# TencentYoutuResearch/ImageMatching-OETR

Hardware: AMD Instinct MI355X
Metric: image-pairs/sec @640x640 (OETR hot path: feature correlation + overlap regression, features resident in HBM) (higher is better)
Workload: dtype f32 (3xf16-split operands, fp32 accumulate); 1 GPU; BASELINE configs[1]: batch=8 pairs/GPU, 640x640 -> 20x20 tokens/image, C=256, 8 enc + 2 dec layers, f32_split_f16; pairs_per_gpu=8, global_pairs=8, streams=3, world_size=1, gpu_max_hw_queues=4, encoder_tile_rows=64, tail_mode=direct form (throughput setting for overlapped streams), parallelism=pairs sharded over 1 rank(s); all-gather of boxes only

## Files before the change

imagematching_oetr_amd/csrc/api.hip:

```cpp
#include <math.h>
#include <stdlib.h>
#include <string.h>

#include <atomic>
#include <string>
#include <vector>

#include "../../include/oetr_hip.h"
#include "../../include/oetr_tail_share.h"
#include "common.h"

using namespace oetr;

constexpr int OETR_PREREDUCE_MIN_TOKENS = 768;
constexpr int OETR_DIRECT_TAIL_MIN_ROWS = 16000;

namespace {

thread_local std::string g_err;

oetr_status fail(oetr_status st, const std::string& msg) {
  g_err = msg;
  return st;
}
// ... 103 lines not shown
  std::vector<hipEvent_t> ev;
  std::vector<int> kid;
  int used = 0;
  int dropped = 0;
};

struct oetr_ctx {
  oetr_trace* trace = nullptr;
  int device = 0;
  int mode = GM_SPLIT;
  int kv_prereduce = -1;
  int tail_share = -1;
  mutable std::atomic<int> enc_grid{0};
  mutable int dec_fault = 0;
  int dec_split = 0;
  int tail_mode = 0;
  int policy = 0;
  int enc_tile = 0;
  int attn_full = 0;
  int num_cus = 256;
  float* dev = nullptr;
  size_t dev_floats = 0;
  EncLayerDev enc[OETR_N_ENC];
  DecKVDev dkv;
  DecLayerDev dec[OETR_N_DEC];
  const float* qe[2];
  const float *dec_tgt1, *dec_q0, *dec_qkv1;
  HeadsDev heads;
};

struct oetr_neck_ctx {
  oetr_trace* trace = nullptr;
  int device = 0;
  int num_cus = 256;
  int conv_rows = 0;
  float* dev = nullptr;
  const f32x4 *proj_wh[2], *proj_wl[2];
  const float *proj_b, *ln_w, *ln_b;
  const f32x4 *conv_wh[3], *conv_wl[3];
  const f32x4 *conv_wh_rw[3], *conv_wl_rw[3];
  int conv_kernel = 0;
  const float* conv_b[3];
  const f32x4 *out_wh, *out_wl;
  const float* out_b;
};

namespace {

#ifdef OETR_PHASE_TIMING
long long* g_tbuf = nullptr;
#endif

struct Workspace {
  float *x, *qp, *pos, *kvp[2], *ksp[2], *att0, *z0, *dkv1, *dks1, *conv_out, *gn_part, *sm_part, *hs,
      *logits, *cxy, *tlbr, *convp, *kbuf[2], *vt[2], *kvr, *ksr;
  uint32_t* flags;
  size_t bytes;
};

bool make_geom(int n, int hf1, int wf1, int hf2, int wf2, Geom* g) {
  if (n <= 0 || hf1 <= 0 || wf1 <= 0 || hf2 <= 0 || wf2 <= 0) return false;
  const long L1 = (long)hf1 * wf1, L2 = (long)hf2 * wf2;
  if (L1 > OETR_MAX_TOKENS || L2 > OETR_MAX_TOKENS) return false;
  if ((long)n * (L1 + L2) > (1L << 30) / C) return false;
  g->N = n;
  g->L[0] = (int)L1; g->L[1] = (int)L2;
  g->hf[0] = hf1; g->wf[0] = wf1; g->hf[1] = hf2; g->wf[1] = wf2;
  g->nt[0] = (g->L[0] + TM - 1) / TM; g->nt[1] = (g->L[1] + TM - 1) / TM;
  g->row0[0] = 0; g->row0[1] = n * g->L[0];
  g->prow0[0] = 0; g->prow0[1] = g->L[0];
  g->tile0[0] = 0; g->tile0[1] = n * g->nt[0];
  g->ntiles = n * (g->nt[0] + g->nt[1]);
  g->rows = n * (g->L[0] + g->L[1]);
  return true;
}

int encoder_tile_rows(const oetr_ctx* h, const Geom& g) {
  if (!gm_half(h->mode) || h->attn_full) return TM;
  const int want = h->enc_tile;
  if (want == TM || want == 64) return want;
  return g.ntiles > h->num_cus ? 64 : TM;
}
Geom encoder_geom(const Geom& g, int rows) {
  Geom e = g;
  for (int i = 0; i < 2; ++i) e.nt[i] = (g.L[i] + rows - 1) / rows;
  e.tile0[0] = 0; e.tile0[1] = g.N * e.nt[0];
  e.ntiles = g.N * (e.nt[0] + e.nt[1]);
  return e;
}

Workspace carve(const Geom& g, void* base, bool attn_full = false) {
  Workspace w;
  size_t off = 0;
  auto take = [&](size_t floats) {
    float* p = base ? reinterpret_cast<float*>(static_cast<char*>(base) + off) : nullptr;
    off += (floats * sizeof(float) + 255) & ~size_t(255);
    return p;
  };
  const size_t rows = g.rows, nt = g.ntiles;
  w.flags = reinterpret_cast<uint32_t*>(take(OETR_WORKSPACE_STATUS_BYTES / sizeof(float)));
  w.x = take(rows * C);
  w.qp = take((rows + (size_t)2 * g.N * 64) * C);
  w.pos = take((size_t)(g.L[0] + g.L[1]) * C);
  for (int i = 0; i < 2; ++i) { w.kvp[i] = take(nt * KV_FLOATS); w.ksp[i] = take(nt * C); }
  w.att0 = take(nt * C); w.z0 = take(nt * NH);
  w.dkv1 = take(nt * KV_FLOATS); w.dks1 = take(nt * C);
  w.conv_out = take(rows * C);
  w.gn_part = take(nt * 32 * 2);
  w.sm_part = take(nt * 4);
  w.hs = take((size_t)2 * g.N * C);
  w.logits = take(rows);
  w.cxy = take((size_t)2 * g.N * 2);
  w.tlbr = take((size_t)2 * g.N * 4);
  w.convp = take((size_t)9 * rows * C);
  w.kvr = take((size_t)2 * g.N * KV_FLOATS);
  w.ksr = take((size_t)2 * g.N * C);
  for (int i = 0; i < 2; ++i) {
    w.kbuf[i] = attn_full ? take(rows * C) : nullptr;
    w.vt[i] = attn_full ? take((size_t)g.N * C * TM * (g.nt[0] + g.nt[1])) : nullptr;
  }
  w.bytes = off;
  return w;
}

oetr_status check_ws(const Geom& g, void* ws, size_t ws_bytes, Workspace* out, bool attn_full = false) {
  if (!ws) return fail(OETR_ERR_WORKSPACE, "workspace is NULL");
  if (reinterpret_cast<uintptr_t>(ws) & 255)
    return fail(OETR_ERR_WORKSPACE, "workspace must be 256-byte aligned");
  *out = carve(g, ws, attn_full);
  if (out->bytes > ws_bytes)
    return fail(OETR_ERR_WORKSPACE, "workspace too small: need " + std::to_string(out->bytes) +
                                        " bytes, got " + std::to_string(ws_bytes));
  return OETR_OK;
}

HeatLaunch heat_launch(const oetr_ctx* h, const Geom& g, const Workspace& w, const float* mem1,
                       const float* mem2, const float* hs1, const float* hs2, float* cxy1,
                       float* cxy2, int img_h1, int img_h2) {
  HeatLaunch p;
  p.g = g;
  p.w = h->heads;
  p.mem[0] = mem1; p.mem[1] = mem2;
  p.hs[0] = hs1; p.hs[1] = hs2;
  p.conv_out = w.conv_out;
  p.gn_part = w.gn_part;
  p.sm_part = w.sm_part;
  p.logits = w.logits;
  p.cxy[0] = cxy1; p.cxy[1] = cxy2;
  p.img_h[0] = img_h1; p.img_h[1] = img_h2;
  p.tlbr[0] = p.tlbr[1] = nullptr;
  p.box[0] = p.box[1] = nullptr;
  p.img_w[0] = p.img_w[1] = 0;
  p.flags = w.flags;
  p.publish = nullptr;
  p.force_staged_conv = h->tail_mode == 3;
  p.convp_units = 9;
  p.mask[0] = p.mask[1] = nullptr;
  return p;
}

oetr_status check_masks(const oetr_ctx* h, const float* mask1, const float* mask2, bool encoder) {
  if (!mask1 && !mask2) return OETR_OK;
  if (!mask1 || !mask2) return fail(OETR_ERR_BAD_ARG, "masks: pass both mask1 and mask2, or neither");
  if (encoder && ((h->mode != GM_SPLIT && h->mode != GM_F32) || h->attn_full))
    return fail(OETR_ERR_UNSUPPORTED, "masks: built for OETR_DTYPE_F32_SPLIT_F16, OETR_DTYPE_F32_SPLIT_QK16 and OETR_DTYPE_F32 with linear attention "
                                      "(the reference's FullAttention turns a masked query row into NaN, "
                                      "linear_attention.py:74-81)");
  return OETR_OK;
}

struct Scoped {
  oetr_trace* t; hipStream_t s; int slot;
  Scoped(oetr_trace* tr, hipStream_t s_, int kid) : t(tr), s(s_), slot(-1) {
// ... 26 lines not shown
      const int units = 9 * g.N * ((g.L[0] + RT - 1) / RT + (g.L[1] + RT - 1) / RT);
      const int avail = h->num_cus - images * DEC_SPLIT_K;
      const int upi = std::max(3, (units + avail - 1) / avail);
      fits = upi <= 9;
      if (fits) d.convp_units = upi;
    } else {
      fits = images * DEC_SPLIT_K + g.ntiles <= h->num_cus;
    }
  }
  if (h->dec_split == DEC_SPLIT_K && d.convp_units == 9 && beside_convp && gm_half(h->mode)) d.convp_units = 3;
  d.ksplit = (h->dec_split == DEC_SPLIT_K || (h->dec_split == 0 && fits)) && images <= DEC_SPLIT_MAX_IMAGES
                 ? DEC_SPLIT_K : 1;
  d.flags = w.flags;
  d.xch_epoch = w.flags + STATUS_EPOCH_WORD;
  d.xch = reinterpret_cast<unsigned long long*>(reinterpret_cast<char*>(w.flags) + STATUS_XCH_OFFSET);
  d.tbuf = nullptr;
  d.dbg = 0;
  if (d.ksplit == DEC_SPLIT_K && h->dec_fault) { d.dbg = DEC_DBG_FAULT; h->dec_fault = 0; }
#ifdef OETR_PHASE_TIMING
  d.tbuf = g_tbuf ? g_tbuf + 16 * 4096 : nullptr;
#endif
  return d;
}

oetr_status run_correlation(oetr_ctx* h, const Geom& g, const Workspace& w, const float* feat1,
                            const float* feat2, const float* pos1, const float* pos2,
                            int enc_layers, hipStream_t s, bool with_decoder = true,
                            bool resident = false, const float* mask1 = nullptr,
                            const float* mask2 = nullptr) {
  EncLaunch p;
  memset(&p, 0, sizeof(p));
  if (!resident) {
    p.feat_nchw[0] = feat1; p.feat_nchw[1] = feat2;
    p.pos_nchw[0] = pos1; p.pos_nchw[1] = pos2;
    p.pos_out = w.pos;
  }
  p.tile_rows = encoder_tile_rows(h, g);
  p.g = encoder_geom(g, p.tile_rows);
  p.tail_share = h->tail_share != 0;
  p.attn_full = h->attn_full;
  h->enc_grid.store(encoder_workgroups(p, h->mode), std::memory_order_relaxed);
#ifdef OETR_ABLATE
  { const char* e = getenv("OETR_ABLATE"); p.dbg = e ? atoi(e) : 0; }
#endif
#ifdef OETR_PHASE_TIMING
  {
    static long long* tb = nullptr;
    if (!tb) (void)hipMalloc(&tb, sizeof(long long) * 16 * 65536);
    p.tbuf = tb;
    g_tbuf = tb;
  }
#endif
  p.x = w.x; p.qp = w.qp; p.pos = w.pos;
  p.mask[0] = mask1; p.mask[1] = mask2;
  p.flags = w.flags;
  p.policy = h->policy;
  for (int i = 0; i < 2; ++i) p.lpad[i] = g.nt[i] * TM;
  p.vt_off[0] = 0; p.vt_off[1] = (size_t)g.N * C * p.lpad[0];
  p.kbuf_out = w.kbuf[0]; p.vt_out = w.vt[0];
  p.a = h->enc[0];
  p.kv_out = w.kvp[0]; p.ks_out = w.ksp[0];
  int prereduce = h->attn_full ? 0 : h->kv_prereduce;
  if (prereduce < 0) prereduce = (g.L[0] >= OETR_PREREDUCE_MIN_TOKENS || g.L[1] >= OETR_PREREDUCE_MIN_TOKENS) ? 1 : 0;
  TRACED(h, s, K_ENC_A, launch_encoder(p, false, 0, h->mode, s));
  p.feat_nchw[0] = p.feat_nchw[1] = p.pos_nchw[0] = p.pos_nchw[1] = nullptr;
  for (int l = 0; l < enc_layers; ++l) {
    p.b = h->enc[l];
    p.b_cross = l & 1;
    p.kv_in = w.kvp[l & 1]; p.ks_in = w.ksp[l & 1];
    p.kv_reduced = 0;
    if (prereduce == 1) {
      TRACED(h, s, K_KV_REDUCE, launch_kv_reduce(p.g, w.kvp[l & 1], w.ksp[l & 1], w.kvr, w.ksr, s));
      p.kv_in = w.kvr; p.ks_in = w.ksr;
      p.kv_reduced = 1;
    }
    p.kbuf_in = w.kbuf[l & 1]; p.vt_in = w.vt[l & 1];
    int tail;
    if (l + 1 == OETR_N_ENC) {
      tail = 1;
      p.d = h->dkv;
      p.att0_out = w.att0; p.z0_out = w.z0; p.dkv1_out = w.dkv1; p.dks1_out = w.dks1;
      p.dec_q0 = h->dec_q0;
    } else if (l + 1 < enc_layers) {
      tail = 0;
      p.a = h->enc[l + 1];
      p.kv_out = w.kvp[(l + 1) & 1]; p.ks_out = w.ksp[(l + 1) & 1];
      p.kbuf_out = w.kbuf[(l + 1) & 1]; p.vt_out = w.vt[(l + 1) & 1];
    } else {
      tail = 2;
    }
    TRACED(h, s, tail == 0 ? K_ENC_BA : tail == 1 ? K_ENC_BDEC : K_ENC_B,
           launch_encoder(p, true, tail, h->mode, s));
  }
  if (enc_layers == OETR_N_ENC && with_decoder) {
    DecLaunch d = dec_launch(h, g, w);
    TRACED(h, s, K_DECODER, launch_decoder(d, s));
  }
  return OETR_OK;
}

oetr_status check_weight(const char* name, const float* w, size_t n, bool f16_range) {
  for (size_t i = 0; i < n; ++i) {
    const float a = fabsf(w[i]);
    if (!(a <= 3.4028234e38f))
      return fail(OETR_ERR_UNSUPPORTED, std::string(name) + ": non-finite weight at index " + std::to_string(i));
    if (f16_range && a >= 65504.0f)
// ... 1034 lines not shown
```

imagematching_oetr_amd/csrc/common.h:

```cpp
#pragma once
#include <hip/hip_runtime.h>
#include <stdint.h>

#include <string>
#include <type_traits>

#include "../../include/oetr_hip.h"

namespace oetr {

constexpr int C = 256;
constexpr int NH = 8;
constexpr int HD = 32;
constexpr int FF = 512;
constexpr int TM = 32;
constexpr int LDA = C + 4;
constexpr int LDH = FF + 4;
constexpr int NTHREADS = 256;
constexpr int KV_FLOATS = NH * HD * HD;
constexpr float LN_EPS = 1e-5f;
constexpr float ATTN_EPS = 1e-6f;
constexpr int MAX_TOKENS = 10000;


// ... 759 lines not shown
    NoEpi none;
    gemm_epi<KTOT, P, HAS_NEXT, NKTOT, SITE, NSITE, TR>(A, W, Wl, nt0, ks0, lane, acc, nW, nWl, nnt0,
                                                        nks0, none);
  }
  template <int KTOT, int P, bool HAS_NEXT, int NKTOT, int SITE = SITE_FULL, int NSITE = SITE_FULL,
            bool TR = false, class EPI, int RP>
  __device__ __forceinline__ void gemm_epi(const PlanesT<M, RP>& A, const f32x4* W, const f32x4* Wl, int nt0,
                                           int ks0, int lane, f32x16 (&acc)[NMT], const f32x4* nW,
                                           const f32x4* nWl, int nnt0, int nks0, EPI& epi) {
    const size_t off = ((size_t)nt0 * (KTOT / 16) + ks0) * 64;
    const size_t noff = ((size_t)nnt0 * (NKTOT / 16) + nks0) * 64;
    const int a_off = (lane & 31) * LDAH + 8 * (lane >> 5);
    const _Float16* ah_ptr = A.h + a_off;
    const _Float16* al_ptr = A.l + a_off;
    AStep a[2];
    load_a<SITE>(a[0], ah_ptr, al_ptr, 0);
    f32x16 cross[NMT];
#pragma unroll
    for (int mt = 0; mt < NMT; ++mt) cross[mt] = f32x16{0};
    step<P, HAS_NEXT, 0, EPI, TR, SITE, NSITE>(ah_ptr, al_ptr, W + off, Wl + off,
                                               HAS_NEXT ? nW + noff : nullptr,
                                               HAS_NEXT ? nWl + noff : nullptr, a, acc, cross, epi);
    if constexpr (TWO && SITE != SITE_HI) {
#pragma unroll
      for (int mt = 0; mt < NMT; ++mt)
#pragma unroll
        for (int r = 0; r < 16; ++r) acc[mt][r] = fmaf(cross[mt][r], SPLIT_INV, acc[mt][r]);
    }
  }
};
typedef WStream2T<GM_SPLIT> WStream2;

#endif

int set_last_error(int status, const char* msg);
oetr_status entry_fail(const char* entry, oetr_status status, const std::string& msg);
oetr_status entry_hip(const char* entry, hipError_t e, const char* what);
hipError_t clear_i32(int32_t* p, int64_t n, hipStream_t s);
struct EncLayerDev {
  const f32x4 *wq, *wk, *wv, *wmerge, *w1, *w2;
  const f32x4 *wq_l, *wk_l, *wv_l, *wmerge_l, *w1_l, *w2_l;
  const float *lnq_w, *lnq_b, *lnkv_w, *lnkv_b, *ln2_w, *ln2_b;
};
struct DecKVDev {
  const f32x4 *wk[2], *wv[2];
  const f32x4 *wk_l[2], *wv_l[2];
  const float *bk[2], *bv[2];
};

struct EncLaunch {
  Geom g;
  float* x;
  float* qp;
  const float* pos;
  const float* kv_in;
  const float* ks_in;
  float* kv_out;
  float* ks_out;
  float* att0_out;
  float* z0_out;
  float* dkv1_out;
  float* dks1_out;
  const float* dec_q0;
  EncLayerDev b;
  EncLayerDev a;
  DecKVDev d;
  int attn_full;
  const float* kbuf_in;
  const float* vt_in;
  float* kbuf_out;
  float* vt_out;
  int lpad[2];
  size_t vt_off[2];
  int tile_rows;
  int nwg;
  int tail_share;
  int b_cross;
  int kv_reduced;
  int policy;
  int dbg;
  long long* tbuf;
  uint32_t* flags;
  const float* feat_nchw[2];
  const float* pos_nchw[2];
  float* pos_out;
  const float* mask[2];
};

hipError_t launch_encoder(const EncLaunch& p, bool has_b, int tail, int mode, hipStream_t s);
int encoder_workgroups(const EncLaunch& p, int mode);
hipError_t launch_kv_reduce(const Geom& g, const float* kvp, const float* ksp, float* kvr, float* ksr,
                            hipStream_t s);

struct MhaDev {
  const float *wq_t, *wk_t, *wv_t, *wm_t;
  const float *bq, *bk, *bv;
};
struct DecLayerDev {
  MhaDev self_attn, cross;
  const float *w1_t, *w2_t;
  const float *n1w, *n1b, *n2w, *n2b, *n3w, *n3b;
};
struct DecLaunch {
  Geom g;
  DecLayerDev layer[2];
  const float* qe[2];
// ... 123 lines not shown
```

imagematching_oetr_amd/csrc/encoder.hip:

```cpp
#include <type_traits>

#include "common.h"


#ifndef OETR_SOAK_AMP
#define OETR_SOAK_AMP 0
#endif
#ifndef OETR_SPLIT_STATE
#define OETR_SPLIT_STATE 1
#endif

namespace oetr {

constexpr int S0_OFF = 0;
constexpr int S1_OFF = S0_OFF + TM * LDA;
constexpr int H_OFF = S1_OFF + TILE_FLOATS;
constexpr int KSUM_OFF = H_OFF + HID_FLOATS;
constexpr int Z_OFF = KSUM_OFF + C;
constexpr int LNP_OFF = Z_OFF + TM * NH;
constexpr int SMEM_FLOATS = LNP_OFF + 6 * C;

template <int NW>
struct EncCfg {
  static constexpr int NT = 8 / NW;
// ... 747 lines not shown
    };
    row_tile(std::integral_constant<int, 0>{});
    if constexpr (NMT == 2) {
      if (two) row_tile(std::integral_constant<int, 1>{});
    }
#if OETR_SOAK_AMP & 2
    __builtin_amdgcn_s_setprio(0);
#endif
#pragma unroll
    for (int r = 0; r < 16; ++r) kv[r] = fmaf(c1[r], SPLIT_INV, kv[r]);
  } else {
    auto row_tile = [&](auto MT_) {
      constexpr int mt = decltype(MT_)::value;
      auto operands = [&](int r, float& k, float& v) {
        float m;
        if constexpr (MASKED) m = msk_s[32 * mt + crow(r, half)];
        else if constexpr (LO16) m = (r >= 8 && 32 * mt + crow(r, 0) < nv2) ? 1.0f : 0.0f;
        else m = 32 * mt + crow(r, 0) < nv2 ? 1.0f : 0.0f;
        const float x = accK[mt][r];
        k = (elu1(x)) * m;
        ksum += k;
        v = accV[mt][r] * (inv_len * m);
      };
      float kc, vc;
      operands(0, kc, vc);
#pragma unroll
      for (int r = 0; r < 16; ++r) {
        float kn = 0.f, vn = 0.f;
        if (r + 1 < 16) operands(r + 1, kn, vn);
        kv = __builtin_amdgcn_mfma_f32_32x32x2f32(kc, vc, kv, 0, 0, 0);
        __builtin_amdgcn_sched_barrier(0);
        kc = kn; vc = vn;
      }
    };
    row_tile(std::integral_constant<int, 0>{});
    if constexpr (NMT == 2) {
      if (two) row_tile(std::integral_constant<int, 1>{});
    }
  }
  ksum += __shfl_xor(ksum, 32, 64);
}
__device__ __forceinline__ void kv_state_write(const f32x16& kv, float ksum, int lane, int wave,
                                               float* __restrict__ kv_out,
                                               float* __restrict__ ks_out, int slot) {
  f32x4* dst = reinterpret_cast<f32x4*>(kv_out) + ((size_t)slot * NH + wave) * 4 * 64;
#pragma unroll
  for (int q = 0; q < 4; ++q) {
    f32x4 o = {kv[4 * q], kv[4 * q + 1], kv[4 * q + 2], kv[4 * q + 3]};
    store16(reinterpret_cast<float*>(dst), (q * 64 + (unsigned)lane) * 16u, o);
  }
  if (lane < 32) (ks_out + (size_t)slot * C + wave * HD)[(unsigned)lane] = ksum;
}

struct EncWg { int n, side, t_idx; bool shared; };
__device__ __forceinline__ EncWg enc_wg(const EncLaunch& p) {
  const Geom& g = p.g;
  const int logical = xcd_remap(blockIdx.x, p.nwg);
  const int f0 = g.nt[0] - p.tail_share;
  const int per = f0 + g.nt[1];
  EncWg w;
  w.n = logical / per;
  const int rem = logical - w.n * per;
  w.shared = p.tail_share != 0 && rem == per - 1;
  w.side = !w.shared && rem >= f0;
  w.t_idx = w.shared ? f0 : w.side ? rem - f0 : rem;
  return w;
}

template <bool HAS_B, int TAIL, int MODE, int POL, int ROWS, int RTW = RT, bool MASKED = false>
__device__ __forceinline__ void encoder64_body(const EncLaunch& p, float* smem) {
  constexpr int NMT = RTW / 32, THREADS = 512, TPR = THREADS / RTW, F4 = 64 / TPR;
  using L2 = E2<RTW>;
  using SP = SitePolicy<POL>;
  float* R1f = smem + L2::R1;
  float* R2f = smem + L2::R2;
  Range rg;
  const PlanesT<MODE, RTW> P1(R1f, &rg), P2(R2f, &rg);
  float* Xf = HAS_B ? R2f : R1f;
  float* ksum_s = smem + L2::KSUM;
  float* lnp_s = smem + L2::LNP;
  float* lnx_s = smem + L2::LNX;
  float* ksum2_s = lnx_s + 32 * LNX_LD;
  using WS = WStream2T<MODE, ROWS, NMT>;
  WS ws;
  constexpr int P_MERGE = 0;
  constexpr int P_1A = WS::adv(P_MERGE), P_1B = WS::adv(P_1A), P_2A = WS::adv(P_1B), P_2B = WS::adv(P_2A);
  constexpr int P_T0 = HAS_B ? WS::adv(P_2B) : 0;
  constexpr int P_T1 = WS::adv(P_T0), P_T2 = WS::adv(P_T1), P_T3 = WS::adv(P_T2);

  const Geom& g = p.g;
  const int tid = threadIdx.x, lane = tid & 63, wave = __builtin_amdgcn_readfirstlane(tid >> 6);
  const int half = lane >> 5, col = lane & 31;
  const int wcol = 32 * wave;
  const int lrow = tid / TPR, lpart = tid % TPR;

  const EncWg wg = enc_wg(p);
  const int n = wg.n, side = wg.side, t_idx = wg.t_idx;
  const int L = g.L[side];
  const int l0 = t_idx * RTW;
  const int nvalid = min(RTW, L - l0);
  const size_t row_base = (size_t)g.row0[side] + (size_t)n * L + l0;
  const int slot = g.tile0[side] + n * g.nt[side] + t_idx;
  const size_t qrow_base = (size_t)slot * RTW;
  const bool nchw = !HAS_B && p.feat_nchw[0] != nullptr;
  ws.set_rows(nvalid);
  ws.set_lane(lane);

  constexpr bool Seg2 = ROWS == 1 && RTW == RT;
  static_assert(!Seg2 || gm_f16_range(MODE), "one-row-tile body: two-plane modes");
  const int r2 = Seg2 && wg.shared ? g.L[1] - (g.nt[1] - 1) * RTW : 0;
  const bool sh = r2 != 0;
  const int side2 = sh ? 1 : side, Lb = g.L[side2], l02 = sh ? (g.nt[1] - 1) * RTW : l0;
  const size_t row_base2 = sh ? (size_t)g.row0[1] + (size_t)n * Lb + l02 : row_base;
  const int slot2 = sh ? g.tile0[1] + n * g.nt[1] + g.nt[1] - 1 : slot;
  auto seg_of = [&](int r) { return Seg2 && sh && r >= 16; };
  auto seg_row = [&](int r) { return seg_of(r) ? min(r - 16, r2 - 1) : min(r, nvalid - 1); };
  auto x_row = [&](int r) { return (seg_of(r) ? row_base2 : row_base) + seg_row(r); };
  auto pos_row = [&](int r) { return (seg_of(r) ? g.prow0[1] + l02 : g.prow0[side] + l0) + seg_row(r); };
  const bool lane_seg = seg_of(col);

  stage_ln_params<THREADS, HAS_B, TAIL>(lnp_s, p, tid);
  const f32x4* pos = reinterpret_cast<const f32x4*>(p.pos + (size_t)pos_row(lrow) * C) + lpart;

  f32x16 xacc[NMT];
  PHASE_STAMP(p, 0);
  if (!HAS_B) PHASE_STAMP(p, 13);

  if (HAS_B) {
    const int ss = p.b_cross ? 1 - side : side;
    const int S_len = g.L[ss];
    const int nts = p.kv_reduced ? 1 : g.nt[ss];
    const int src_slot0 = p.kv_reduced ? ss * g.N + n : g.tile0[ss] + n * g.nt[ss];

    f32x4 kvB[4];
    auto reduce_state = [&](f32x4 (&kvB)[4], float* ksum_s, int nts, int src_slot0) {
#pragma unroll
    for (int q = 0; q < 4; ++q) kvB[q] = f32x4{0.f, 0.f, 0.f, 0.f};
    {
      constexpr int KVR = 7;
      const unsigned ln = lane, kl = tid & (C - 1);
      const f32x4* kvp = reinterpret_cast<const f32x4*>(p.kv_in) + ((size_t)src_slot0 * NH + wave) * 256;
      const float* ksp = p.ks_in + (size_t)src_slot0 * C;
      float ks = 0.f;
      if (nts == 1) {
#pragma unroll
        for (int e = 0; e < 4; ++e) kvB[e] = kvp[e * 64 + ln];
        ks = ksp[kl];
      } else
      for (int ti0 = 0; ti0 < nts; ti0 += KVR) {
        f32x4 tmp[KVR][4];
        float kt[KVR];
#pragma unroll
        for (int u = 0; u < KVR; ++u) {
          const int ti = min(ti0 + u, nts - 1);
#pragma unroll
          for (int e = 0; e < 4; ++e) tmp[u][e] = kvp[(size_t)ti * (NH * 256) + e * 64 + ln];
          kt[u] = ksp[(size_t)ti * C + kl];
        }
#pragma unroll
        for (int u = 0; u < KVR; ++u)
          if (ti0 + u < nts) {
#pragma unroll
            for (int e = 0; e < 4; ++e) kvB[e] += tmp[u][e];
            ks += kt[u];
          }
      }
      if (tid < C) ksum_s[tid] = ks;
    }
    };
    reduce_state(kvB, ksum_s, nts, src_slot0);
    const int ss2 = p.b_cross ? 1 - side2 : side2;
    const int S_len2 = g.L[ss2];
    f32x4 kvB2[4];
    if constexpr (Seg2) {
      if (sh) {
        reduce_state(kvB2, ksum2_s, p.kv_reduced ? 1 : g.nt[ss2], p.kv_reduced ? ss2 * g.N + n : g.tile0[ss2] + n * g.nt[ss2]);
      } else {
#pragma unroll
        for (int q = 0; q < 4; ++q) kvB2[q] = f32x4{0.f, 0.f, 0.f, 0.f};
        if (tid < C) ksum2_s[tid] = 0.f;
      }
    }
    ws.template prime<C, P_MERGE, SP::MERGE>(p.b.wmerge, p.b.wmerge_l, wave, 0, lane);
    f32x4 qfrag[NMT][4];
    {
      const f32x4* qf = reinterpret_cast<const f32x4*>(p.qp + qrow_base * C) + (size_t)wave * NMT * 4 * 64;
#pragma unroll
      for (int mt = 0; mt < NMT; ++mt)
#pragma unroll
        for (int u = 0; u < 4; ++u) qfrag[mt][u] = qf[(mt * 4 + u) * 64 + (unsigned)lane];
    }
#pragma unroll
    for (int mt = 0; mt < NMT; ++mt) {
      const float* xr = p.x + x_row(32 * mt + col) * C + wcol + 4 * half;
#pragma unroll
      for (int g4 = 0; g4 < 4; ++g4) {
        const f32x4 v = *reinterpret_cast<const f32x4*>(xr + 8 * g4);
#pragma unroll
        for (int i = 0; i < 4; ++i) xacc[mt][4 * g4 + i] = v[i];
      }
    }
    __syncthreads();
    PHASE_STAMP(p, 1);

    {
      f32x4 kvh[2], kvl[2], ksh[2], ksl[2];
      f32x4 kvh2[2], kvl2[2], ksh2[2], ksl2[2];
      const float inv_S = 1.0f / (float)S_len;
      (void)inv_S;
      if constexpr (gm_f16_range(MODE)) {
#pragma unroll
        for (int s2 = 0; s2 < 2; ++s2) {
          split8(kvB[2 * s2], kvB[2 * s2 + 1], kvh[s2], kvl[s2], rg);
          const float* kr = ksum_s + wave * HD + 4 * half + 16 * s2;
          split8(*reinterpret_cast<const f32x4*>(kr) * inv_S, *reinterpret_cast<const f32x4*>(kr + 8) * inv_S,
                 ksh[s2], ksl[s2], rg);
          if constexpr (Seg2) {
            const float inv_S2 = 1.0f / (float)S_len2;
            split8(kvB2[2 * s2], kvB2[2 * s2 + 1], kvh2[s2], kvl2[s2], rg);
            const float* kr2 = ksum2_s + wave * HD + 4 * half + 16 * s2;
            split8(*reinterpret_cast<const f32x4*>(kr2) * inv_S2, *reinterpret_cast<const f32x4*>(kr2 + 8) * inv_S2,
                   ksh2[s2], ksl2[s2], rg);
          }
        }
      }
#pragma unroll
      for (int mt = 0; mt < NMT; ++mt) {
        if (mt == 1 && !ws.two()) break;
        f32x16 macc = {0}, zacc = {0};
        if constexpr (gm_f16_range(MODE)) {
          f32x16 c1 = {0}, cz = {0};
#pragma unroll
          for (int s2 = 0; s2 < 2; ++s2) {
            const f32x4 qh = qfrag[mt][2 * s2], ql = qfrag[mt][2 * s2 + 1];
            mma16_split3(kvh[s2], kvl[s2], qh, ql, macc, c1);
            mma16_split3(ksh[s2], ksl[s2], qh, ql, zacc, cz);
          }
#pragma unroll
          for (int r = 0; r < 16; ++r) macc[r] = fmaf(c1[r], SPLIT_INV, macc[r]);
          zacc[0] = fmaf(cz[0], SPLIT_INV, zacc[0]);
          if constexpr (Seg2) {
            f32x16 macc2 = {0}, zacc2 = {0}, c2 = {0}, cz2 = {0};
#pragma unroll
            for (int s2 = 0; s2 < 2; ++s2) {
              const f32x4 qh = qfrag[mt][2 * s2], ql = qfrag[mt][2 * s2 + 1];
              mma16_split3(kvh2[s2], kvl2[s2], qh, ql, macc2, c2);
              mma16_split3(ksh2[s2], ksl2[s2], qh, ql, zacc2, cz2);
            }
#pragma unroll
            for (int r = 0; r < 16; ++r) macc[r] = lane_seg ? fmaf(c2[r], SPLIT_INV, macc2[r]) : macc[r];
            zacc[0] = lane_seg ? fmaf(cz2[0], SPLIT_INV, zacc2[0]) : zacc[0];
          }
        } else {
#pragma unroll
// ... 47 lines not shown
        float msum = 0.f, qsum = 0.f;
#pragma unroll
        for (int i = 0; i < 8; ++i) { msum += t[i][0] + t[i][2]; qsum += t[i][1] + t[i][3]; }
        const float mean = msum * (1.0f / 16.0f);
        float dev = 0.f;
#pragma unroll
        for (int i = 0; i < 8; ++i) {
          const float d0 = t[i][0] - mean, d1 = t[i][2] - mean;
          dev = fmaf(d0, d0, dev);
          dev = fmaf(d1, d1, dev);
        }
        const float rstd = 1.0f / sqrtf((qsum + 16.0f * dev) * (1.0f / C) + LN_EPS);
#pragma unroll
        for (int g4 = 0; g4 < 4; ++g4) {
          const int c0 = wcol + 8 * g4 + 4 * half;
          const f32x4 gw = *reinterpret_cast<const f32x4*>(lnp_s + c0), gb = *reinterpret_cast<const f32x4*>(lnp_s + C + c0);
          f32x4 y;
#pragma unroll
          for (int i = 0; i < 4; ++i) y[i] = (xacc[mt][4 * g4 + i] - mean) * rstd * gw[i] + gb[i];
          P1.put4(32 * mt + col, c0, y);
        }
      }
    }
    __syncthreads();

    PHASE_STAMP(p, 4);
    {
      constexpr int SNEXT = TAIL == 0 ? SP::Q : SP::DEC_K;
      constexpr bool XTR = true;
      f32x16 haccA[NMT] = {}, haccB[NMT] = {};
      ws.template gemm<C, P_1A, true, C, SP::MLP1, SP::MLP1, true>(P1, p.b.w1, p.b.w1_l, wave, 0, lane, haccA,
                                                                   p.b.w1, p.b.w1_l, 8 + wave, 0);
      const bool two = ws.two();
      auto gelu_to = [&](const PlanesT<MODE, RTW>& dst, const f32x16 (&h)[NMT]) {
        return [&, two](auto CI_) {
          constexpr int CI = decltype(CI_)::value, mt = NMT == 2 ? CI / 8 : 0, g4 = NMT == 2 ? (CI % 8) / 2 : CI / 4;
          if constexpr (CI % (NMT == 2 ? 2 : 4) == 0) {
            if (mt == 1 && !two) return;
            const f32x4 ge = gelu_erf4(f32x4{h[mt][4 * g4], h[mt][4 * g4 + 1], h[mt][4 * g4 + 2], h[mt][4 * g4 + 3]});
            dst.template put4<site_act_lo(SP::MLP2)>(32 * mt + col, wcol + 8 * g4 + 4 * half, ge);
          }
        };
      };
      auto epiA = gelu_to(P2, haccA);
      ws.template gemm_epi<C, P_1B, true, FF, SP::MLP1, SP::MLP2, true>(P1, p.b.w1, p.b.w1_l, 8 + wave, 0, lane,
                                                                        haccB, p.b.w2, p.b.w2_l, wave, 0, epiA);
      __syncthreads();
      PHASE_STAMP(p, 5);
      auto epiB = gelu_to(P1, haccB);
      ws.template gemm_epi<FF, P_2A, true, FF, SP::MLP2, SP::MLP2, XTR>(P2, p.b.w2, p.b.w2_l, wave, 0, lane, xacc,
                                                                        p.b.w2, p.b.w2_l, wave, 16, epiB);
      __syncthreads();
      PHASE_STAMP(p, 6);
      PHASE_STAMP(p, 7);
      ws.template gemm<FF, P_2B, (TAIL != 2), C, SP::MLP2, SNEXT, XTR>(P1, p.b.w2, p.b.w2_l, wave, 16, lane, xacc,
                                                                       TAIL == 0 ? p.a.wq : p.d.wk[0],
                                                                       TAIL == 0 ? p.a.wq_l : p.d.wk_l[0], wave, 0);
    }
#pragma unroll
    for (int mt = 0; mt < NMT; ++mt)
#pragma unroll
      for (int g4 = 0; g4 < 4; ++g4)
        *reinterpret_cast<f32x4*>(Xf + (32 * mt + col) * LDA + wcol + 8 * g4 + 4 * half) =
            f32x4{xacc[mt][4 * g4], xacc[mt][4 * g4 + 1], xacc[mt][4 * g4 + 2], xacc[mt][4 * g4 + 3]};
    __syncthreads();
#pragma unroll
    for (int i = 0; i < RTW / 8; ++i) {
      const int r = wave + 8 * i;
      if (seg_of(r) ? r - 16 < r2 : r < nvalid)
        store16(p.x + x_row(r) * C, 16u * (unsigned)lane,
                                    *reinterpret_cast<const f32x4*>(Xf + r * LDA + 4 * lane));
    }
    PHASE_STAMP(p, 8);
    if (TAIL == 2) { range_report<MODE>(rg, p.flags); return; }
  } else {
    if (nchw) {
      if constexpr (Seg2) {
        const int r = tid % RTW;
        const bool s2 = seg_of(r);
        const int Ls = s2 ? Lb : L, tok = (s2 ? l02 : l0) + seg_row(r);
        load_rows_nchw<THREADS, RTW>(R1f, p.feat_nchw[s2 ? 1 : side] + (size_t)n * C * Ls + tok, Ls, tid);
        load_rows_nchw<THREADS, RTW>(R2f, p.pos_nchw[s2 ? 1 : side] + tok, Ls, tid);
      } else {
      load_tile_nchw<THREADS, RTW>(R1f, p.feat_nchw[side] + (size_t)n * C * L + l0, L, nvalid, tid);
      load_tile_nchw<THREADS, RTW>(R2f, p.pos_nchw[side] + l0, L, nvalid, tid);
      }
    } else {
#pragma unroll
      for (int i = 0; i < (RTW * C / 4) / THREADS; ++i) {
        const int idx = tid + THREADS * i;
        const int r = idx >> 6, c4 = idx & 63;
        *reinterpret_cast<f32x4*>(R1f + r * LDA + 4 * c4) =
            reinterpret_cast<const f32x4*>(p.x + x_row(r) * C)[c4];
      }
    }
    if (TAIL == 0) ws.template prime<C, P_T0, SP::Q>(p.a.wq, p.a.wq_l, wave, 0, lane);
    if (TAIL == 1) ws.template prime<C, P_T0, SP::DEC_K>(p.d.wk[0], p.d.wk_l[0], wave, 0, lane);
    __syncthreads();
    if (nchw) {
      if constexpr (Seg2) {
#pragma unroll
        for (int i = 0; i < 32 / 8; ++i) {
          const int r = wave + 8 * i;
          if (seg_of(r) ? r - 16 < r2 : r < nvalid) {
            reinterpret_cast<f32x4*>(p.x + x_row(r) * C)[lane] = *reinterpret_cast<const f32x4*>(R1f + r * LDA + 4 * lane);
            if (n == 0)
              reinterpret_cast<f32x4*>(p.pos_out + (size_t)pos_row(r) * C)[lane] = *reinterpret_cast<const f32x4*>(R2f + r * LDA + 4 * lane);
          }
        }
      } else {
      store_tile_tokens<THREADS, RTW>(p.x + row_base * C, R1f, nvalid, tid);
      if (n == 0) store_tile_tokens<THREADS, RTW>(p.pos_out + (size_t)(g.prow0[side] + l0) * C, R2f, nvalid, tid);
      }
    }
    PHASE_STAMP(p, 14);
  }

  if constexpr (MASKED && TAIL != 2 && Seg2) {
    if (tid < 32) {
      const bool s2 = seg_of(tid);
      const bool ok = s2 ? tid - 16 < r2 : tid < nvalid;
      const float m = ok ? p.mask[s2 ? 1 : side][(size_t)n * (s2 ? Lb : L) + (s2 ? l02 : l0) + seg_row(tid)] : 0.f;
      lnx_s[tid] = s2 ? 0.f : m;
      lnx_s[32 + tid] = s2 ? m : 0.f;
    }
  } else if constexpr (MASKED && TAIL != 2) {
    if (tid < RTW) lnx_s[tid] = tid < nvalid ? p.mask[side][(size_t)n * L + l0 + tid] : 0.f;
  }
  if (TAIL == 0) {
    {
      f32x4 xn[F4], ps[F4];
      if (!HAS_B && nchw) {
        const f32x4* pl = reinterpret_cast<const f32x4*>(R2f + lrow * LDA) + lpart;
#pragma unroll
        for (int i = 0; i < F4; ++i) ps[i] = pl[i * TPR];
      } else {
#pragma unroll
        for (int i = 0; i < F4; ++i) ps[i] = pos[i * TPR];
      }
      ln_rows<TPR, F4>(Xf, tid, xn, 0);
      __syncthreads();
      const f32x4* qw = reinterpret_cast<const f32x4*>(lnp_s + 2 * C) + lpart;
      const f32x4* qb = reinterpret_cast<const f32x4*>(lnp_s + 3 * C) + lpart;
      const f32x4* kw = reinterpret_cast<const f32x4*>(lnp_s + 4 * C) + lpart;
      const f32x4* kb = reinterpret_cast<const f32x4*>(lnp_s + 5 * C) + lpart;
#pragma unroll
      for (int i = 0; i < F4; ++i) {
        P1.template put4<site_act_lo(SP::Q)>(lrow, 4 * (i * TPR + lpart), (xn[i] * qw[i * TPR] + qb[i * TPR]) + ps[i]);
        P2.template put4<site_act_lo(SP::K) || site_act_lo(SP::V)>(lrow, 4 * (i * TPR + lpart),
                                                                   (xn[i] * kw[i * TPR] + kb[i * TPR]) + ps[i]);
      }
    }
    __syncthreads();
    PHASE_STAMP(p, 9);
    f32x16 accQ[NMT] = {};
    ws.template gemm<C, P_T0, true, C, SP::Q, SP::K, true>(P1, p.a.wq, p.a.wq_l, wave, 0, lane, accQ, p.a.wk,
                                                           p.a.wk_l, wave, 0);
    PHASE_STAMP(p, 10);
    f32x16 accK[NMT] = {}, accV[NMT] = {};
    {
      f32x4* qf = reinterpret_cast<f32x4*>(p.qp + qrow_base * C) + (size_t)wave * NMT * 4 * 64;
      const bool two = ws.two();
      u32x4 qhi = {0, 0, 0, 0}, qlo = {0, 0, 0, 0};
      auto qepi = [&](auto CI_) {
        constexpr int CI = decltype(CI_)::value, mt = NMT == 2 ? CI / 8 : 0, pr = NMT == 2 ? CI % 8 : CI / 2;
        constexpr int s2 = pr / 4, j = pr % 4;
        if constexpr (NMT == 1 && CI % 2 == 1) return;
        if (mt == 1 && !two) return;
        const float qmask = MASKED ? lnx_s[32 * (Seg2 ? (int)lane_seg : mt) + col] : 1.0f;
        const float a = MASKED ? elu1(accQ[mt][2 * pr]) * qmask : elu1(accQ[mt][2 * pr]);
        const float b = MASKED ? elu1(accQ[mt][2 * pr + 1]) * qmask : elu1(accQ[mt][2 * pr + 1]);
        if constexpr (MODE == GM_BF16) {
          if constexpr (pr % 2 == 0) { qhi[0] = __builtin_bit_cast(uint32_t, a); qhi[1] = __builtin_bit_cast(uint32_t, b); }
          else {
            qhi[2] = __builtin_bit_cast(uint32_t, a); qhi[3] = __builtin_bit_cast(uint32_t, b);
            store16(reinterpret_cast<float*>(qf), ((mt * 4 + pr / 2) * 64 + (unsigned)lane) * 16u,
                                        __builtin_bit_cast(f32x4, qhi));
          }
        } else {
          uint32_t h, l;
          cvt_planes2<GM_SPLIT>(a, b, h, l, rg);
          qhi[j] = h; qlo[j] = l;
          if constexpr (j == 3) {
            store16(reinterpret_cast<float*>(qf), ((mt * 4 + 2 * s2) * 64 + (unsigned)lane) * 16u,
                                        __builtin_bit_cast(f32x4, qhi));
            store16(reinterpret_cast<float*>(qf), ((mt * 4 + 2 * s2 + 1) * 64 + (unsigned)lane) * 16u,
                                        __builtin_bit_cast(f32x4, qlo));
          }
        }
      };
      ws.template gemm_epi<C, P_T1, true, C, SP::K, SP::V>(P2, p.a.wk, p.a.wk_l, wave, 0, lane, accK, p.a.wv,
                                                           p.a.wv_l, wave, 0, qepi);
    }
    ws.template gemm<C, P_T2, false, C, SP::V>(P2, p.a.wv, p.a.wv_l, wave, 0, lane, accV, nullptr, nullptr,
                                               0, 0);
    PHASE_STAMP(p, 11);
    f32x16 kv;
    float ksum;
    kv_state_64<MODE, NMT, MASKED>(accK, accV, L, nvalid, half, ws.two(), kv, ksum, rg, lnx_s);
    kv_state_write(kv, ksum, lane, wave, p.kv_out, p.ks_out, slot);
    if constexpr (Seg2) {
      kv_state_64<MODE, NMT, MASKED, true>(accK, accV, Lb, 16 + r2, half, false, kv, ksum, rg, lnx_s + 32);
      if (sh) kv_state_write(kv, ksum, lane, wave, p.kv_out, p.ks_out, slot2);
    }
    PHASE_STAMP(p, 12);
  } else if (TAIL == 1) {
    float bias_k[2], bias_v[2];
#pragma unroll
    for (int dl = 0; dl < 2; ++dl) {
      bias_k[dl] = p.d.bk[dl][wcol + col];
      bias_v[dl] = p.d.bv[dl][wcol + col];
// ... 228 lines not shown
```

Before: 33850 image-pairs/s.

## Keep encoder residual and positional tiles in MFMA fragment layout between layers

Adds workspace buffers that hold the residual stream and positional encodings in per-wave MFMA accumulator fragment order. Encoder layers load and store the residual directly as register fragments instead of going through row-major global rows and the LDS tile. The LayerNorm feeding the next layer is computed from the register fragments with a two-stage partial mean/variance reduction through LDS. Mask staging into LDS is moved later, and an extra barrier is added in the masked path. This cuts LDS round trips and strided global traffic, at the cost of extra workspace, a second residual copy, and more register pressure.

```diff
diff --git a/imagematching_oetr_amd/csrc/api.hip b/imagematching_oetr_amd/csrc/api.hip
--- a/imagematching_oetr_amd/csrc/api.hip
+++ b/imagematching_oetr_amd/csrc/api.hip
@@ -179,7 +179,7 @@
 #endif
 
 struct Workspace {
-  float *x, *qp, *pos, *kvp[2], *ksp[2], *att0, *z0, *dkv1, *dks1, *conv_out, *gn_part, *sm_part, *hs,
+  float *x, *qp, *xf, *posf, *pos, *kvp[2], *ksp[2], *att0, *z0, *dkv1, *dks1, *conv_out, *gn_part, *sm_part, *hs,
       *logits, *cxy, *tlbr, *convp, *kbuf[2], *vt[2], *kvr, *ksr;
   uint32_t* flags;
   size_t bytes;
@@ -246,6 +246,8 @@
     w.kbuf[i] = attn_full ? take(rows * C) : nullptr;
     w.vt[i] = attn_full ? take((size_t)g.N * C * TM * (g.nt[0] + g.nt[1])) : nullptr;
   }
+  w.xf = take((rows + (size_t)2 * g.N * 64) * C);
+  w.posf = take((size_t)(g.L[0] + g.L[1] + 2 * 64) * C);
   w.bytes = off;
   return w;
 }
@@ -378,6 +380,7 @@
   }
 #endif
   p.x = w.x; p.qp = w.qp; p.pos = w.pos;
+  p.xf = w.xf; p.posf = w.posf;
   p.mask[0] = mask1; p.mask[1] = mask2;
   p.flags = w.flags;
   p.policy = h->policy;
diff --git a/imagematching_oetr_amd/csrc/common.h b/imagematching_oetr_amd/csrc/common.h
--- a/imagematching_oetr_amd/csrc/common.h
+++ b/imagematching_oetr_amd/csrc/common.h
@@ -835,6 +835,8 @@
   Geom g;
   float* x;
   float* qp;
+  float* xf;
+  float* posf;
   const float* pos;
   const float* kv_in;
   const float* ks_in;
diff --git a/imagematching_oetr_amd/csrc/encoder.hip b/imagematching_oetr_amd/csrc/encoder.hip
--- a/imagematching_oetr_amd/csrc/encoder.hip
+++ b/imagematching_oetr_amd/csrc/encoder.hip
@@ -823,6 +823,44 @@
   if (lane < 32) (ks_out + (size_t)slot * C + wave * HD)[(unsigned)lane] = ksum;
 }
 
+template <int NMT>
+__device__ __forceinline__ void xfrag_store(float* __restrict__ tile, const f32x16 (&x)[NMT], int wave, int lane, bool two) {
+  float* base = tile + (size_t)wave * (NMT * 4 * 64 * 4);
+#pragma unroll
+  for (int mt = 0; mt < NMT; ++mt) {
+    if (mt == 1 && !two) break;
+#pragma unroll
+    for (int g4 = 0; g4 < 4; ++g4)
+      store16(base, ((mt * 4 + g4) * 64 + (unsigned)lane) * 16u,
+              f32x4{x[mt][4 * g4], x[mt][4 * g4 + 1], x[mt][4 * g4 + 2], x[mt][4 * g4 + 3]});
+  }
+}
+template <int NMT>
+__device__ __forceinline__ void xfrag_load(f32x16 (&x)[NMT], const float* __restrict__ tile, int wave, int lane, bool two) {
+  const f32x4* src = reinterpret_cast<const f32x4*>(tile) + (size_t)wave * (NMT * 4 * 64);
+#pragma unroll
+  for (int mt = 0; mt < NMT; ++mt) {
+    if (mt == 1 && !two) { x[mt] = f32x16{0}; break; }
+#pragma unroll
+    for (int g4 = 0; g4 < 4; ++g4) {
+      const f32x4 v = src[(mt * 4 + g4) * 64 + (unsigned)lane];
+#pragma unroll
+      for (int i = 0; i < 4; ++i) x[mt][4 * g4 + i] = v[i];
+    }
+  }
+}
+template <int NMT>
+__device__ __forceinline__ void xfrag_from_lds(f32x16 (&x)[NMT], const float* S, int wcol, int lane) {
+#pragma unroll
+  for (int mt = 0; mt < NMT; ++mt)
+#pragma unroll
+    for (int g4 = 0; g4 < 4; ++g4) {
+      const f32x4 v = *reinterpret_cast<const f32x4*>(S + (32 * mt + (lane & 31)) * LDA + wcol + 8 * g4 + 4 * (lane >> 5));
+#pragma unroll
+      for (int i = 0; i < 4; ++i) x[mt][4 * g4 + i] = v[i];
+    }
+}
+
 struct EncWg { int n, side, t_idx; bool shared; };
 __device__ __forceinline__ EncWg enc_wg(const EncLaunch& p) {
   const Geom& g = p.g;
@@ -893,7 +931,10 @@
   stage_ln_params<THREADS, HAS_B, TAIL>(lnp_s, p, tid);
   const f32x4* pos = reinterpret_cast<const f32x4*>(p.pos + (size_t)pos_row(lrow) * C) + lpart;
 
+  const size_t pos_tile = (size_t)((side ? g.nt[0] : 0) + t_idx) * RTW;
+
   f32x16 xacc[NMT];
+  f32x16 pacc[NMT];
   PHASE_STAMP(p, 0);
   if (!HAS_B) PHASE_STAMP(p, 13);
 
@@ -961,16 +1002,7 @@
 #pragma unroll
         for (int u = 0; u < 4; ++u) qfrag[mt][u] = qf[(mt * 4 + u) * 64 + (unsigned)lane];
     }
-#pragma unroll
-    for (int mt = 0; mt < NMT; ++mt) {
-      const float* xr = p.x + x_row(32 * mt + col) * C + wcol + 4 * half;
-#pragma unroll
-      for (int g4 = 0; g4 < 4; ++g4) {
-        const f32x4 v = *reinterpret_cast<const f32x4*>(xr + 8 * g4);
-#pragma unroll
-        for (int i = 0; i < 4; ++i) xacc[mt][4 * g4 + i] = v[i];
-      }
-    }
+    xfrag_load<NMT>(xacc, p.xf + qrow_base * C, wave, lane, ws.two());
     __syncthreads();
     PHASE_STAMP(p, 1);
 
@@ -1124,11 +1156,16 @@
                                                                         p.b.w2, p.b.w2_l, wave, 16, epiB);
       __syncthreads();
       PHASE_STAMP(p, 6);
+      if (TAIL == 0) PHASE_STAMP(p, 15);
       PHASE_STAMP(p, 7);
+      if constexpr (TAIL == 0) xfrag_load<NMT>(pacc, p.posf + pos_tile * C, wave, lane, ws.two());
       ws.template gemm<FF, P_2B, (TAIL != 2), C, SP::MLP2, SNEXT, XTR>(P1, p.b.w2, p.b.w2_l, wave, 16, lane, xacc,
                                                                        TAIL == 0 ? p.a.wq : p.d.wk[0],
                                                                        TAIL == 0 ? p.a.wq_l : p.d.wk_l[0], wave, 0);
     }
+    if constexpr (TAIL == 0) {
+      xfrag_store<NMT>(p.xf + qrow_base * C, xacc, wave, lane, ws.two());
+    } else {
 #pragma unroll
     for (int mt = 0; mt < NMT; ++mt)
 #pragma unroll
@@ -1142,6 +1179,7 @@
       if (seg_of(r) ? r - 16 < r2 : r < nvalid)
         store16(p.x + x_row(r) * C, 16u * (unsigned)lane,
                                     *reinterpret_cast<const f32x4*>(Xf + r * LDA + 4 * lane));
+    }
     }
     PHASE_STAMP(p, 8);
     if (TAIL == 2) { range_report<MODE>(rg, p.flags); return; }
@@ -1164,6 +1202,8 @@
         const int r = idx >> 6, c4 = idx & 63;
         *reinterpret_cast<f32x4*>(R1f + r * LDA + 4 * c4) =
             reinterpret_cast<const f32x4*>(p.x + x_row(r) * C)[c4];
+        if (TAIL == 0)
+          *reinterpret_cast<f32x4*>(R2f + r * LDA + 4 * c4) = reinterpret_cast<const f32x4*>(p.pos + (size_t)pos_row(r) * C)[c4];
       }
     }
     if (TAIL == 0) ws.template prime<C, P_T0, SP::Q>(p.a.wq, p.a.wq_l, wave, 0, lane);
@@ -1175,60 +1215,106 @@
         for (int i = 0; i < 32 / 8; ++i) {
           const int r = wave + 8 * i;
           if (seg_of(r) ? r - 16 < r2 : r < nvalid) {
-            reinterpret_cast<f32x4*>(p.x + x_row(r) * C)[lane] = *reinterpret_cast<const f32x4*>(R1f + r * LDA + 4 * lane);
+            if (TAIL != 0)
+              reinterpret_cast<f32x4*>(p.x + x_row(r) * C)[lane] = *reinterpret_cast<const f32x4*>(R1f + r * LDA + 4 * lane);
             if (n == 0)
               reinterpret_cast<f32x4*>(p.pos_out + (size_t)pos_row(r) * C)[lane] = *reinterpret_cast<const f32x4*>(R2f + r * LDA + 4 * lane);
           }
         }
       } else {
-      store_tile_tokens<THREADS, RTW>(p.x + row_base * C, R1f, nvalid, tid);
+      if (TAIL != 0) store_tile_tokens<THREADS, RTW>(p.x + row_base * C, R1f, nvalid, tid);
       if (n == 0) store_tile_tokens<THREADS, RTW>(p.pos_out + (size_t)(g.prow0[side] + l0) * C, R2f, nvalid, tid);
       }
     }
+    if constexpr (TAIL == 0) {
+      xfrag_from_lds<NMT>(xacc, R1f, wcol, lane);
+      xfrag_from_lds<NMT>(pacc, R2f, wcol, lane);
+      xfrag_store<NMT>(p.xf + qrow_base * C, xacc, wave, lane, ws.two());
+      if (n == 0) xfrag_store<NMT>(p.posf + pos_tile * C, pacc, wave, lane, ws.two());
+    }
     PHASE_STAMP(p, 14);
   }
 
+  float msk1 = 0.f, msk2 = 0.f;
   if constexpr (MASKED && TAIL != 2 && Seg2) {
     if (tid < 32) {
       const bool s2 = seg_of(tid);
       const bool ok = s2 ? tid - 16 < r2 : tid < nvalid;
       const float m = ok ? p.mask[s2 ? 1 : side][(size_t)n * (s2 ? Lb : L) + (s2 ? l02 : l0) + seg_row(tid)] : 0.f;
-      lnx_s[tid] = s2 ? 0.f : m;
-      lnx_s[32 + tid] = s2 ? m : 0.f;
+      msk1 = s2 ? 0.f : m;
+      msk2 = s2 ? m : 0.f;
     }
   } else if constexpr (MASKED && TAIL != 2) {
-    if (tid < RTW) lnx_s[tid] = tid < nvalid ? p.mask[side][(size_t)n * L + l0 + tid] : 0.f;
-  }
+    if (tid < RTW) msk1 = tid < nvalid ? p.mask[side][(size_t)n * L + l0 + tid] : 0.f;
+  }
+  auto mask_to_lds = [&]() {
+    if constexpr (MASKED && Seg2) {
+      if (tid < 32) { lnx_s[tid] = msk1; lnx_s[32 + tid] = msk2; }
+    } else if constexpr (MASKED) {
+      if (tid < RTW) lnx_s[tid] = msk1;
+    }
+  };
+  if (TAIL == 1) mask_to_lds();
   if (TAIL == 0) {
     {
-      f32x4 xn[F4], ps[F4];
-      if (!HAS_B && nchw) {
-        const f32x4* pl = reinterpret_cast<const f32x4*>(R2f + lrow * LDA) + lpart;
-#pragma unroll
-        for (int i = 0; i < F4; ++i) ps[i] = pl[i * TPR];
-      } else {
-#pragma unroll
-        for (int i = 0; i < F4; ++i) ps[i] = pos[i * TPR];
-      }
-      ln_rows<TPR, F4>(Xf, tid, xn, 0);
+      int colA = col, halfA = half;
+      asm volatile("" : "+v"(colA), "+v"(halfA));
+#pragma unroll
+      for (int mt = 0; mt < NMT; ++mt) {
+        float sum = 0.f;
+#pragma unroll
+        for (int r = 0; r < 16; ++r) sum += xacc[mt][r];
+        const float pm = sum * (1.0f / 16.0f);
+        float q = 0.f;
+#pragma unroll
+        for (int r = 0; r < 16; ++r) { const float d = xacc[mt][r] - pm; q = fmaf(d, d, q); }
+        *reinterpret_cast<f32x2*>(lnx_s + (32 * mt + colA) * LNX_LD + 2 * (2 * wave + halfA)) = f32x2{pm, q};
+      }
       __syncthreads();
-      const f32x4* qw = reinterpret_cast<const f32x4*>(lnp_s + 2 * C) + lpart;
-      const f32x4* qb = reinterpret_cast<const f32x4*>(lnp_s + 3 * C) + lpart;
-      const f32x4* kw = reinterpret_cast<const f32x4*>(lnp_s + 4 * C) + lpart;
-      const f32x4* kb = reinterpret_cast<const f32x4*>(lnp_s + 5 * C) + lpart;
-#pragma unroll
-      for (int i = 0; i < F4; ++i) {
-        P1.template put4<site_act_lo(SP::Q)>(lrow, 4 * (i * TPR + lpart), (xn[i] * qw[i * TPR] + qb[i * TPR]) + ps[i]);
-        P2.template put4<site_act_lo(SP::K) || site_act_lo(SP::V)>(lrow, 4 * (i * TPR + lpart),
-                                                                   (xn[i] * kw[i * TPR] + kb[i * TPR]) + ps[i]);
-      }
-    }
-    __syncthreads();
+#pragma unroll
+      for (int mt = 0; mt < NMT; ++mt) {
+        if (mt == 1 && !ws.two()) break;
+        const f32x4* pp = reinterpret_cast<const f32x4*>(lnx_s + (32 * mt + colA) * LNX_LD);
+        f32x4 t[8];
+#pragma unroll
+        for (int i = 0; i < 8; ++i) t[i] = pp[i];
+        float msum = 0.f, qsum = 0.f;
+#pragma unroll
+        for (int i = 0; i < 8; ++i) { msum += t[i][0] + t[i][2]; qsum += t[i][1] + t[i][3]; }
+        const float mean = msum * (1.0f / 16.0f);
+        float dev = 0.f;
+#pragma unroll
+        for (int i = 0; i < 8; ++i) {
+          const float d0 = t[i][0] - mean, d1 = t[i][2] - mean;
+          dev = fmaf(d0, d0, dev);
+          dev = fmaf(d1, d1, dev);
+        }
+        const float rstd = 1.0f / sqrtf((qsum + 16.0f * dev) * (1.0f / C) + LN_EPS);
+#pragma unroll
+        for (int g4 = 0; g4 < 4; ++g4) {
+          const int c0 = wcol + 8 * g4 + 4 * halfA;
+          const f32x4 qw = *reinterpret_cast<const f32x4*>(lnp_s + 2 * C + c0), qb = *reinterpret_cast<const f32x4*>(lnp_s + 3 * C + c0);
+          const f32x4 kw = *reinterpret_cast<const f32x4*>(lnp_s + 4 * C + c0), kb = *reinterpret_cast<const f32x4*>(lnp_s + 5 * C + c0);
+          f32x4 yq, yk;
+#pragma unroll
+          for (int i = 0; i < 4; ++i) {
+            const float xn = (xacc[mt][4 * g4 + i] - mean) * rstd;
+            yq[i] = (xn * qw[i] + qb[i]) + pacc[mt][4 * g4 + i];
+            yk[i] = (xn * kw[i] + kb[i]) + pacc[mt][4 * g4 + i];
+          }
+          P1.template put4<site_act_lo(SP::Q)>(32 * mt + colA, c0, yq);
+          P2.template put4<site_act_lo(SP::K) || site_act_lo(SP::V)>(32 * mt + colA, c0, yk);
+        }
+      }
+    }
+    __syncthreads();
+    mask_to_lds();
     PHASE_STAMP(p, 9);
     f32x16 accQ[NMT] = {};
     ws.template gemm<C, P_T0, true, C, SP::Q, SP::K, true>(P1, p.a.wq, p.a.wq_l, wave, 0, lane, accQ, p.a.wk,
                                                            p.a.wk_l, wave, 0);
     PHASE_STAMP(p, 10);
+    if constexpr (MASKED) __syncthreads();
     f32x16 accK[NMT] = {}, accV[NMT] = {};
     {
       f32x4* qf = reinterpret_cast<f32x4*>(p.qp + qrow_base * C) + (size_t)wave * NMT * 4 * 64;
```

Result: no change. 34090 image-pairs/s (median of 6 runs) (+0.7%).
